# Improbable-AI/walk-these-ways

Measured on AMD Instinct MI355X. Metric: env-steps/sec (sim+PPO), higher is better.
Workload: dtype f32

## Files before the change

### include/go1ppo.h

```cpp
#ifndef GO1PPO_H
#define GO1PPO_H
#include <stdint.h>

#ifdef __cplusplus
extern "C" {
#endif

#define GO1PPO_ABI_VERSION 3
#define GO1PPO_MAX_ACTIONS 32

int go1ppo_elu_fwd(void* y, int64_t rows, int cols, int ld, const void* lat, int lat_ld, int npv, const void* wz,
                   int wz_ld, int lat_cols, void* stream);

int go1ppo_elu_bwd(const void* d, int ld_d, const void* h, int ld_h, int64_t rows, int cols, float* bias_grad, void* out,
                   int ld_out, void* stream);

typedef struct {
  const void* mean;
  const void* value;
  const float* std;
  int32_t head_ld, num_actions;
  int64_t rows;
  const int64_t* idx;
  const float* actions;
// ... 102 lines not shown
int go1ppo_opt_prestep_pieces(float* g, int64_t n, const Go1PpoGradPiece* device_pieces, int num_pieces, float gscale, float* partial,
                              float* step, float* lr, const float* kl, float kl_scale, float desired_kl, float lr_min, float lr_max,
                              void* stream);

#define GO1PPO_ADAM_MAX_TRANSPOSES 2
typedef struct {
  int32_t num_transposes, _pad;
  struct { int64_t start; int32_t rows, cols; void* dst; } transpose[GO1PPO_ADAM_MAX_TRANSPOSES];
} Go1PpoAdamExtras;
int go1ppo_opt_adam(float* p, float* g, float* m, float* v, int64_t start0, int64_t count0, int64_t start1,
                    int64_t count1, float gscale, const float* partial, float max_norm, const float* step, const float* lr,
                    float beta1, float beta2, float eps, void* body, int64_t n_body, float* tail, int64_t n_tail, int zero_grad,
                    float* zero_slot, const Go1PpoAdamExtras* extras, void* stream);

int go1ppo_sum_partials(const void* partials, int count, int64_t stride, int64_t rows, int cols, float* out, int zero_rows,
                        int zero_c0, int zero_c1, void* stream);


typedef struct Go1PpoGemmArgs {
  const void* A; const void* B; void* C; const float* bias; const void* H;
  int32_t M, N, K, lda, ldb, ldc, ldh, epilogue, elu_c0, elu_c1;
  int32_t elu_skip_c0, elu_skip_c1;
  int32_t bias_bf16, _pad;
} Go1PpoGemmArgs;
int go1ppo_gemm_nt(const Go1PpoGemmArgs* args, void* stream);
int go1ppo_gemm_nt_pair(const Go1PpoGemmArgs* a, const Go1PpoGemmArgs* b, void* stream);

int go1ppo_wgrad_tn_plan(Go1PpoWgradProblem* problems, int count);
int go1ppo_wgrad_tn_batched(const Go1PpoWgradProblem* device_problems, int count, int total_workgroups, void* stream);

#define GO1PPO_MLP2_MAX_NETS 3
typedef struct {
  void* x;
  const void* W2; const void* b2;
  const void* W3; const void* b3;
  void* z2;
  void* out;
  int64_t rows;
  int32_t ld_x, ld_z2, ld_out, elu_input;
} Go1PpoMlp2Fwd;
int go1ppo_mlp2_fwd(const Go1PpoMlp2Fwd* nets, int count, void* stream);

typedef struct {
  const void* d_out;
  const void* z2; const void* h;
  const void* W2; const void* W3;
  void* d_z2;
  void* d_x;
  int64_t rows;
  int32_t ld_dout, ld_z2, ld_h, ld_dz2, ld_dx, _pad;
} Go1PpoMlp2Bwd;
int go1ppo_mlp2_bwd(const Go1PpoMlp2Bwd* nets, int count, void* stream);

const char* go1ppo_version(void);

#ifdef __cplusplus
}
#endif
#endif
```

### walk-these-ways_amd/csrc/go1ppo.hip

```cpp
#include <hip/hip_runtime.h>
#include <stdint.h>
#include <string.h>
#include "../../include/go1ppo.h"

typedef uint16_t bf16_t;
static_assert(sizeof(Go1PpoAdamExtras) == 56 && sizeof(Go1PpoGemmArgs) == 96 && sizeof(Go1PpoWgradProblem) == 96 && sizeof(Go1PpoGradPiece) == 56, "ctypes mirrors (fused.py) assume these sizes");
typedef __attribute__((ext_vector_type(4))) float f32x4;

__device__ __forceinline__ float bf2f(bf16_t u) { return __uint_as_float(((uint32_t)u) << 16); }
__device__ __forceinline__ bf16_t f2bf(float f) {
  return __builtin_bit_cast(bf16_t, (__bf16)f);
}
struct alignas(16) Bf8 { bf16_t v[8]; };

__device__ __forceinline__ float elu1(float x) {
  float em = x > -1e-3f ? fmaf(0.5f * x, x, x) : __expf(x) - 1.f;
  return x > 0.f ? x : em;
}

typedef __attribute__((ext_vector_type(2))) float f32x2;
typedef __attribute__((ext_vector_type(2))) __bf16 bf16x2_t;
__device__ __forceinline__ Bf8 pack_bf8(const float (&x)[8]) {
  union { Bf8 b; uint32_t u[4]; } r;
#pragma unroll
  for (int e = 0; e < 4; e++) {
    f32x2 v = {x[2 * e], x[2 * e + 1]};
    r.u[e] = __builtin_bit_cast(uint32_t, __builtin_convertvector(v, bf16x2_t));
  }
  return r.b;
}

#ifndef ELU_ROWS
#define ELU_ROWS 4
#endif
template <bool LAT>
__global__ __launch_bounds__(256) void elu_fwd_kernel(bf16_t* y, int rows, int cols, int ld, const bf16_t* lat, int lat_ld,
                                                      int npv, const bf16_t* wz, int wz_ld, int lat_cols) {
  int c0 = (blockIdx.x * 16 + (threadIdx.x & 15)) << 3;
  int r0 = blockIdx.y * (16 * ELU_ROWS) + (threadIdx.x >> 4);
  if (c0 >= cols) return;
  Bf8 v[ELU_ROWS];
#pragma unroll
  for (int u = 0; u < ELU_ROWS; u++) {
    int r = r0 + u * 16;
    if (r < rows) v[u] = *reinterpret_cast<const Bf8*>(y + (int64_t)r * ld + c0);
  }
  float x[ELU_ROWS][8];
#pragma unroll
  for (int u = 0; u < ELU_ROWS; u++)
#pragma unroll
    for (int e = 0; e < 8; e++) x[u][e] = bf2f(v[u].v[e]);
  if (LAT && c0 < lat_cols) {
    if (npv == 2) {
      float w0[8], w1[8];
#pragma unroll
      for (int e = 0; e < 8; e++) {
        const uint32_t p = *reinterpret_cast<const uint32_t*>(wz + (int64_t)(c0 + e) * wz_ld);
        w0[e] = __uint_as_float(p << 16);
        w1[e] = __uint_as_float(p & 0xffff0000u);
// ... 1262 lines not shown
```

### walk-these-ways_amd/csrc/go1ppo_mlp.h

```cpp
#pragma once

#define MLP2_K1 256
#define MLP2_N2 128
#define MLP2_N3 64
#define MLP2_BM 64
#define MLP2_WAVES 16
#define MLP2_THREADS (64 * MLP2_WAVES)
#define MLP2_IMG (128 * 128)

struct Mlp2FwdArgs { Go1PpoMlp2Fwd net[GO1PPO_MLP2_MAX_NETS]; };
struct Mlp2BwdArgs { Go1PpoMlp2Bwd net[GO1PPO_MLP2_MAX_NETS]; };

__device__ __forceinline__ int swz_row(int row) { return row & 15; }
__device__ __forceinline__ int swz_red(int row) { return 2 * ((row & 3) | (((row >> 3) & 1) << 2)); }

template <bool RED>
__device__ __forceinline__ void dma_weights(const bf16_t* W, int rows, int cols, bf16_t* img, int wave, int lane) {
  const int windows = cols >> 7, count = (rows >> 2) * windows;
  for (int idx = wave; idx < count; idx += MLP2_WAVES) {
    const int win = idx % windows, blk = idx / windows;
    const int row = blk * 4 + (lane >> 4);
    const int chunk = (lane & 15) ^ (RED ? swz_red(row) : swz_row(row));
    glds16(W + (int64_t)row * cols + win * 128 + chunk * 8, img + win * MLP2_IMG + blk * 4 * 128);
  }
// ... 174 lines not shown
      f32x4 acc[2] = {f32x4{0.f, 0.f, 0.f, 0.f}, f32x4{0.f, 0.f, 0.f, 0.f}};
#pragma unroll
      for (int kk = 0; kk < MLP2_N3 / 32; kk++) {
        const bf16x8_t w = lds_tr_operand(W3t, kk * 32 * 256 + w3off);
#pragma unroll
        for (int m = 0; m < 2; m++) acc[m] = __builtin_amdgcn_mfma_f32_16x16x32_bf16(w, lds_b128(D3i + (mp + m) * 16 * 128, foff[kk]), acc[m], 0, 0, 0);
      }
      const int k0 = kf2 * 16 + 4 * g;
#pragma unroll
      for (int m = 0; m < 2; m++) {
        const int row = (mp + m) * 16 + r;
        uint2* slot = reinterpret_cast<uint2*>(reinterpret_cast<char*>(D2i) + row * 256 + (((k0 >> 3) ^ swz_row(row)) << 4) + ((k0 >> 2) & 1) * 8);
        float h[4], o4[4];
        unpack_bf4(*slot, h);
#pragma unroll
        for (int e = 0; e < 4; e++) o4[e] = acc[m][e] * (h[e] > 0.f ? 1.f : h[e] + 1.f);
        *slot = pack_bf4(o4);
      }
    }
    __syncthreads();
    {
      f32x4 acc[4];
#pragma unroll
      for (int m = 0; m < 4; m++) acc[m] = f32x4{0.f, 0.f, 0.f, 0.f};
#pragma unroll
      for (int kk = 0; kk < MLP2_N2 / 32; kk++) {
        const bf16x8_t w = lds_tr_operand(w2img, kk * 32 * 256 + w2off);
#pragma unroll
        for (int m = 0; m < 4; m++) acc[m] = __builtin_amdgcn_mfma_f32_16x16x32_bf16(w, lds_b128(D2i + m * 16 * 128, foff[kk]), acc[m], 0, 0, 0);
      }
      const int k0 = (wave & 7) * 16 + 4 * g;
#pragma unroll
      for (int m = 0; m < 4; m++) {
        const int row = m * 16 + r;
        uint2* slot = reinterpret_cast<uint2*>(reinterpret_cast<char*>(Hi + (wave >> 3) * 64 * 128) + row * 256 +
                                               (((k0 >> 3) ^ swz_row(row)) << 4) + ((k0 >> 2) & 1) * 8);
        float h[4], o4[4];
        unpack_bf4(*slot, h);
#pragma unroll
        for (int e = 0; e < 4; e++) o4[e] = acc[m][e] * (h[e] > 0.f ? 1.f : h[e] + 1.f);
        *slot = pack_bf4(o4);
      }
    }
    __syncthreads();
    if (row0 + zrow < N.rows) *reinterpret_cast<uint4*>(dz2 + (row0 + zrow) * N.ld_dz2 + zch * 8) = *reinterpret_cast<const uint4*>(reinterpret_cast<const char*>(D2i) + zslot);
#pragma unroll
    for (int j = 0; j < 2; j++)
      if (row0 + MLP2_HROW(j) < N.rows)
        *reinterpret_cast<uint4*>(dx + (row0 + MLP2_HROW(j)) * N.ld_dx + hch * 8) = *reinterpret_cast<const uint4*>(reinterpret_cast<const char*>(Hi) + MLP2_HSLOT(j));
    __syncthreads();
  }
}

static inline bool aligned8(const void* p) { return (reinterpret_cast<uintptr_t>(p) & 7) == 0; }

extern "C" int go1ppo_mlp2_fwd(const Go1PpoMlp2Fwd* nets, int count, void* stream) {
  if (!nets || count <= 0 || count > GO1PPO_MLP2_MAX_NETS) return -1;
  Mlp2FwdArgs A;
  int64_t max_rows = 0;
  for (int i = 0; i < count; i++) {
    const Go1PpoMlp2Fwd& N = nets[i];
    if (!N.x || !N.W2 || !N.b2 || !N.W3 || !N.b3 || !N.z2 || !N.out || N.rows <= 0) return -1;
    if ((N.ld_x & 7) || (N.ld_z2 & 3) || (N.ld_out & 3) || N.ld_x < MLP2_K1 || N.ld_z2 < MLP2_N2 || N.ld_out < MLP2_N3 || !aligned16(N.x) ||
        !aligned16(N.W2) || !aligned16(N.W3) || !aligned8(N.b2) || !aligned8(N.b3) || !aligned8(N.z2) || !aligned8(N.out))
      return -2;
    A.net[i] = N;
    if (N.rows > max_rows) max_rows = N.rows;
  }
  int64_t wgs = (max_rows + MLP2_BM - 1) / MLP2_BM;
  if (wgs > 256 / count) wgs = 256 / count;
  mlp2_fwd_kernel<<<dim3((unsigned)wgs, count), dim3(MLP2_THREADS), 0, (hipStream_t)stream>>>(A);
  return hipGetLastError() == hipSuccess ? 0 : -9;
}

extern "C" int go1ppo_mlp2_bwd(const Go1PpoMlp2Bwd* nets, int count, void* stream) {
  if (!nets || count <= 0 || count > GO1PPO_MLP2_MAX_NETS) return -1;
  Mlp2BwdArgs A;
  int64_t max_rows = 0;
  for (int i = 0; i < count; i++) {
    const Go1PpoMlp2Bwd& N = nets[i];
    if (!N.d_out || !N.z2 || !N.h || !N.W2 || !N.W3 || !N.d_z2 || !N.d_x || N.rows <= 0) return -1;
    if ((N.ld_dout & 7) || (N.ld_z2 & 7) || (N.ld_h & 7) || (N.ld_dz2 & 7) || (N.ld_dx & 7) || N.ld_dout < MLP2_N3 || N.ld_z2 < MLP2_N2 ||
        N.ld_h < MLP2_K1 || N.ld_dz2 < MLP2_N2 || N.ld_dx < MLP2_K1 || !aligned16(N.d_out) || !aligned16(N.W2) || !aligned16(N.W3) ||
        !aligned16(N.z2) || !aligned16(N.h) || !aligned16(N.d_z2) || !aligned16(N.d_x))
      return -2;
    A.net[i] = N;
    if (N.rows > max_rows) max_rows = N.rows;
  }
  int64_t wgs = (max_rows + MLP2_BM - 1) / MLP2_BM;
  if (wgs > 256 / count) wgs = 256 / count;
  mlp2_bwd_kernel<<<dim3((unsigned)wgs, count), dim3(MLP2_THREADS), 0, (hipStream_t)stream>>>(A);
  return hipGetLastError() == hipSuccess ? 0 : -9;
}
```

### walk-these-ways_amd/go1_gym_learn/ppo_cse/fused.py

```python
import ctypes
import os

import torch

HEAD = 64
_HERE = os.path.dirname(os.path.abspath(__file__))
_LIB_PATH = os.path.normpath(os.path.join(_HERE, "..", "..", "csrc", "libgo1ppo.so"))
_lib = None


class Go1PpoLibraryMissing(RuntimeError):
    pass


class LossArgs(ctypes.Structure):
    _fields_ = [("mean", ctypes.c_void_p), ("value", ctypes.c_void_p), ("std", ctypes.c_void_p),
                ("head_ld", ctypes.c_int32), ("num_actions", ctypes.c_int32), ("rows", ctypes.c_int64),
                ("idx", ctypes.c_void_p), ("actions", ctypes.c_void_p), ("old_mu", ctypes.c_void_p),
                ("old_sigma", ctypes.c_void_p), ("old_logp", ctypes.c_void_p), ("advantages", ctypes.c_void_p),
                ("returns", ctypes.c_void_p), ("old_values", ctypes.c_void_p),
                ("clip_param", ctypes.c_float), ("value_loss_coef", ctypes.c_float), ("entropy_coef", ctypes.c_float),
                ("use_clipped_value_loss", ctypes.c_int32),
                ("d_mean", ctypes.c_void_p), ("d_value", ctypes.c_void_p), ("d_std", ctypes.c_void_p),
                ("d_mean_bias", ctypes.c_void_p), ("d_value_bias", ctypes.c_void_p), ("kl", ctypes.c_void_p),
                ("value_loss", ctypes.c_void_p), ("surrogate_loss", ctypes.c_void_p)]


class WgradProblem(ctypes.Structure):
    _fields_ = [("dz", ctypes.c_void_p), ("h", ctypes.c_void_p), ("dW", ctypes.c_void_p), ("bias_grad", ctypes.c_void_p),
                ("rows", ctypes.c_int64), ("ld_dz", ctypes.c_int32), ("ld_h", ctypes.c_int32), ("n", ctypes.c_int32),
                ("k", ctypes.c_int32), ("ldw", ctypes.c_int32), ("chunk_rows", ctypes.c_int32), ("wg_offset", ctypes.c_int32),
                ("zero_n", ctypes.c_int32), ("zero_k0", ctypes.c_int32), ("zero_k1", ctypes.c_int32),
                ("partials", ctypes.c_void_p), ("partial_stride", ctypes.c_int64)]


class GradPiece(ctypes.Structure):
    _fields_ = [("begin", ctypes.c_int64), ("count", ctypes.c_int64), ("src", ctypes.c_void_p), ("stride", ctypes.c_int64),
                ("kind", ctypes.c_int32), ("slabs", ctypes.c_int32), ("cols", ctypes.c_int32), ("zero_rows", ctypes.c_int32),
                ("zero_c0", ctypes.c_int32), ("zero_c1", ctypes.c_int32)]


class TailLayer(ctypes.Structure):
    _fields_ = [("W", ctypes.c_void_p), ("bias", ctypes.c_void_p), ("out", ctypes.c_void_p), ("n_out", ctypes.c_int32),
                ("k_in", ctypes.c_int32), ("ld_out", ctypes.c_int32), ("elu", ctypes.c_int32)]


class TailNet(ctypes.Structure):
    _fields_ = [("in_", ctypes.c_void_p), ("rows", ctypes.c_int64), ("ld_in", ctypes.c_int32), ("num_layers", ctypes.c_int32),
                ("elu_in", ctypes.c_int32), ("npv", ctypes.c_int32), ("latent", ctypes.c_void_p), ("wz", ctypes.c_void_p),
                ("lat_ld", ctypes.c_int32), ("wz_ld", ctypes.c_int32),
                ("layer", TailLayer * 4)]


class TailArgs(ctypes.Structure):
    _fields_ = [("num_nets", ctypes.c_int32), ("_pad", ctypes.c_int32), ("net", TailNet * 3)]


class Mlp2Fwd(ctypes.Structure):
    _fields_ = [(n, ctypes.c_void_p) for n in ("x", "W2", "b2", "W3", "b3", "z2", "out")] + [("rows", ctypes.c_int64)] + \
               [(n, ctypes.c_int32) for n in ("ld_x", "ld_z2", "ld_out", "elu_input")]


class Mlp2Bwd(ctypes.Structure):
    _fields_ = [(n, ctypes.c_void_p) for n in ("d_out", "z2", "h", "W2", "W3", "d_z2", "d_x")] + [("rows", ctypes.c_int64)] + \
               [(n, ctypes.c_int32) for n in ("ld_dout", "ld_z2", "ld_h", "ld_dz2", "ld_dx", "_pad")]


MLP2_DIMS = (256, 128, 64)


class GemmArgs(ctypes.Structure):
    _fields_ = [("A", ctypes.c_void_p), ("B", ctypes.c_void_p), ("C", ctypes.c_void_p), ("bias", ctypes.c_void_p),
                ("H", ctypes.c_void_p)] + [(n, ctypes.c_int32) for n in
                                           ("M", "N", "K", "lda", "ldb", "ldc", "ldh", "epilogue", "elu_c0", "elu_c1", "elu_skip_c0", "elu_skip_c1", "bias_bf16", "_pad")]


class _AdamTranspose(ctypes.Structure):
    _fields_ = [("start", ctypes.c_int64), ("rows", ctypes.c_int32), ("cols", ctypes.c_int32), ("dst", ctypes.c_void_p)]


class AdamExtras(ctypes.Structure):
    _fields_ = [("num_transposes", ctypes.c_int32), ("_pad", ctypes.c_int32), ("transpose", _AdamTranspose * 2)]


EXPORTED_SYMBOLS = ["go1ppo_mlp2_fwd", "go1ppo_mlp2_bwd", "go1ppo_gemm_nt", "go1ppo_gemm_nt_pair", "go1ppo_sum_partials", "go1ppo_wgrad_tn_plan", "go1ppo_wgrad_tn_batched", "go1ppo_tail_fwd", "go1ppo_elu_fwd", "go1ppo_elu_bwd", "go1ppo_loss", "go1ppo_mse", "go1ppo_wgrad", "go1ppo_wgrad_plan",
                    "go1ppo_wgrad_batched", "go1ppo_act",
                    "go1ppo_store_step", "go1ppo_ring_snapshot", "go1ppo_ring_step", "go1ppo_ring_gather", "go1ppo_gae", "go1ppo_normalize", "go1ppo_opt_partials", "go1ppo_opt_prestep",
                    "go1ppo_opt_prestep_pieces", "go1ppo_grad_reduce", "go1ppo_opt_adam", "go1ppo_version"]


def load_library(path=None):
    global _lib
    if _lib is not None and path is None:
        return _lib
    p = path or _LIB_PATH
    if not os.path.exists(p):
        raise Go1PpoLibraryMissing(f"{p} not found: run `python -c 'import __graft_entry__ as g; g.build()'` "
                                   "(hipcc --offload-arch=gfx950); the fused PPO update has no CPU fallback")
    L = ctypes.CDLL(p)
    vp, i32, i64 = ctypes.c_void_p, ctypes.c_int, ctypes.c_int64
    L.go1ppo_elu_fwd.argtypes = [vp, i64, i32, i32, vp, i32, i32, vp, i32, i32, vp]
    L.go1ppo_elu_bwd.argtypes = [vp, i32, vp, i32, i64, i32, vp, vp, i32, vp]
    L.go1ppo_loss.argtypes = [ctypes.POINTER(LossArgs), vp]
    L.go1ppo_mse.argtypes = [vp, i32, vp, i32, vp, i64, i64, i32, vp, vp, vp, vp, vp]
    L.go1ppo_wgrad.argtypes = [vp, i32, vp, i32, i64, i32, i32, vp, i32, vp, vp]
    L.go1ppo_wgrad_plan.argtypes = [ctypes.POINTER(WgradProblem), i32]
    L.go1ppo_tail_fwd.argtypes = [ctypes.POINTER(TailArgs), vp]
    L.go1ppo_gemm_nt.argtypes = [ctypes.POINTER(GemmArgs), vp]
    L.go1ppo_gemm_nt_pair.argtypes = [ctypes.POINTER(GemmArgs), ctypes.POINTER(GemmArgs), vp]
    L.go1ppo_sum_partials.argtypes = [vp, i32, i64, i64, i32, vp, i32, i32, i32, vp]
    L.go1ppo_mlp2_fwd.argtypes = [ctypes.POINTER(Mlp2Fwd), i32, vp]
    L.go1ppo_mlp2_bwd.argtypes = [ctypes.POINTER(Mlp2Bwd), i32, vp]
    L.go1ppo_wgrad_batched.argtypes = [vp, i32, i32, vp]
    L.go1ppo_wgrad_tn_plan.argtypes = [ctypes.POINTER(WgradProblem), i32]
    L.go1ppo_wgrad_tn_batched.argtypes = [vp, i32, i32, vp]
    f32 = ctypes.c_float
    L.go1ppo_act.argtypes = [vp, vp, i32, vp, i32, i64, vp, vp, vp, vp, vp, vp, vp]
    L.go1ppo_store_step.argtypes = [vp, vp, vp, vp, vp, f32, i64, vp, vp, vp, vp]
    L.go1ppo_ring_snapshot.argtypes = [vp, i64, i64, i32, i32, vp, vp]
    L.go1ppo_ring_step.argtypes = [vp, vp, vp, vp, i64, i32, i32, i32, i32, vp, vp, vp, vp]
    L.go1ppo_ring_gather.argtypes = [vp, vp, vp, i64, i64, i32, i32, i32, i32, vp, vp]
    L.go1ppo_gae.argtypes = [vp, vp, vp, vp, i32, i64, f32, f32, vp, vp, vp, vp]
    L.go1ppo_normalize.argtypes = [vp, i64, vp, vp]
    L.go1ppo_opt_partials.argtypes = []
    L.go1ppo_opt_prestep.argtypes = [vp, i64, f32, vp, vp, vp, vp, f32, f32, f32, f32, vp]
    L.go1ppo_opt_prestep_pieces.argtypes = [vp, i64, vp, i32, f32, vp, vp, vp, vp, f32, f32, f32, f32, vp]
    L.go1ppo_grad_reduce.argtypes = [vp, vp, i32, vp]
    L.go1ppo_opt_adam.argtypes = [vp, vp, vp, vp, i64, i64, i64, i64, f32, vp, f32, vp, vp, f32, f32, f32, vp, i64, vp, i64, i32, vp,
                                  ctypes.POINTER(AdamExtras), vp]
    for name in EXPORTED_SYMBOLS[:-1]:
        getattr(L, name).restype = ctypes.c_int
    L.go1ppo_version.restype = ctypes.c_char_p
    if path is None:
        _lib = L
    return L


def _stream():
    return torch.cuda.current_stream().cuda_stream


def _chk(rc, what):
    if rc != 0:
        raise RuntimeError(f"{what} failed with code {rc}")


def _ptr(t):
    return None if t is None else t.data_ptr()


def _ld(t):
    assert t.dim() == 2 and t.stride(1) == 1
    return t.stride(0)


def gemm_args(a, b, c, bias=None, elu=None, elu_bwd_of=None, elu_skip=None):
    g = GemmArgs()
    g.A, g.B, g.C, g.bias, g.H = a.data_ptr(), b.data_ptr(), c.data_ptr(), _ptr(bias), _ptr(elu_bwd_of)
    g.M, g.N, g.K, g.lda, g.ldb, g.ldc = a.shape[0], b.shape[0], a.shape[1], _ld(a), _ld(b), _ld(c)
    assert b.shape[1] == g.K and tuple(c.shape) == (g.M, g.N) and (elu is None or elu_bwd_of is None)
    assert a.dtype == b.dtype == c.dtype == torch.bfloat16 and (bias is None or bias.dtype in (torch.float32, torch.bfloat16))
    g.bias_bf16 = int(bias is not None and bias.dtype == torch.bfloat16)
    if elu_bwd_of is not None:
        assert elu_bwd_of.shape == c.shape and elu_bwd_of.dtype == torch.bfloat16
        g.epilogue, g.ldh = 2, _ld(elu_bwd_of)
# ... 10 lines not shown
    _chk(lib.go1ppo_gemm_nt(ctypes.byref(g), _stream()), "go1ppo_gemm_nt")
    return c


def gemm_nt_pair(lib, first, second):
    ga, gb = gemm_args(**first), gemm_args(**second)
    _chk(lib.go1ppo_gemm_nt_pair(ctypes.byref(ga), ctypes.byref(gb), _stream()), "go1ppo_gemm_nt_pair")


class FusedNet:

    def __init__(self, policy, body, grad, M, lib, with_grad, two_streams=True, fused_tails=None):
        assert body.dtype == torch.bfloat16 and body.is_cuda
        self.pol, self.M, self.lib = policy, M, lib
        dev = body.device
        self.P = {name: policy._block(body, name) for name, _ in policy.blocks}
        self.G = {name: policy._block(grad, name) for name, _ in policy.blocks} if grad is not None else None
        self.nd, self.na, self.nc = policy.first
        self.n1 = self.nd + self.na + self.nc
        self.depth = {n: len(l) for n, l in policy.nets.items()}
        bf = dict(device=dev, dtype=torch.bfloat16)
        self.Y1 = torch.zeros(M, self.n1, **bf)
        self.Y1d = torch.zeros(M, self.nd, **bf)
        self.Z = {n: {li: torch.zeros(M, self.P[f"{n}.{li}.W"].shape[0], **bf) for li in range(1, d)}
                  for n, d in self.depth.items()}
        assert policy.npv <= HEAD and self.P["Wz"].shape == (self.na, HEAD)
        self._recording, self._batched, self._plans = None, False, {}
        self._grad = grad
        self.defer_grad_sum = False
        self._rec_pieces, self._slab_ws, self._last_pieces = None, {}, {}
        self._wgrad_tn = M % 64 == 0
        self._tails = self._tails_ad = None
        if fused_tails is None:
            fused_tails = M <= int(os.environ.get("GO1_FUSED_TAILS_MAX_ROWS", "2048"))
        self._elu_on_load = not with_grad
        if fused_tails and self._fused_tails_ok():
            nd, na = self.nd, self.na
            eol = self._elu_on_load
            self._tails = (self._tail_args([("adaptation", self.Y1[:, :nd])], with_grad, elu_in=eol),
                           self._tail_args([("actor", self.Y1[:, nd:nd + na]), ("critic", self.Y1[:, nd + na:])], with_grad, elu_in=eol,
                                           latent_for="actor" if eol else None))
            self._tails_ad = self._tail_args([("adaptation", self.Y1d)], with_grad)
        self._mlp2 = (self._tails is None and os.environ.get("GO1_MLP2", "1") == "1" and self.nd == MLP2_DIMS[0] and
                      all(self.depth[n] >= 3 and tuple(self.P[f"{n}.{self.depth[n] - 2}.W"].shape) == (MLP2_DIMS[1], MLP2_DIMS[0])
                          and tuple(self.P[f"{n}.{self.depth[n] - 1}.W"].shape) == (MLP2_DIMS[2], MLP2_DIMS[1]) for n in self.depth)
                      and self.depth["adaptation"] == 3 and self.depth["actor"] == 4 and self.depth["critic"] == 4)
        self._mlp2_cache = {}
        na1, nc1 = int(self.P["actor.1.W"].shape[0]), int(self.P["critic.1.W"].shape[0])
        nt_ok = all(v % 64 == 0 for v in (na1, nc1, self.na, self.n1 - self.nd - self.na)) and \
            all(self.P[k].data_ptr() % 16 == 0 for k in ("actor.1.b", "critic.1.b", "actor.1.W", "critic.1.W"))
        pair_ok = nt_ok and na1 == nc1 and self.na == self.n1 - self.nd - self.na
        self._l1_nt = nt_ok
        self._pair = pair_ok
        self._side = torch.cuda.Stream(device=dev) if two_streams else None
        if with_grad:
            self.X = torch.zeros(M, policy.Kp, **bf)
            self.dH1 = {"adaptation": torch.zeros(M, self.nd, **bf), "actor": torch.zeros(M, self.na, **bf),
                        "critic": torch.zeros(M, self.nc, **bf)}
            self.dY1 = torch.zeros(M, self.n1, **bf)
            self.dZ = {n: {li: torch.zeros_like(z) for li, z in zs.items()} for n, zs in self.Z.items()}
            w1_split = next((b for b in (M // 6144, 4, 2) if b >= 2 and M % b == 0 and (M // b) % 64 == 0), 1)
            self._w1_tmp = torch.zeros(w1_split, self.n1, policy.Kp, **bf)
            self._dgrad_nt = self._mlp2 and nt_ok
            self._WT = {n: torch.zeros(self.P[f"{n}.1.W"].shape[1], self.P[f"{n}.1.W"].shape[0], **bf) for n in ("actor", "critic")} \
                if self._dgrad_nt else None
            self._wt_by_optimizer = False
            self.priv_mask = (self.nd + self.na, policy.K + 1, policy.K + 1 + policy.npv)

    def _elu(self, y, lat=None, lat_cols=0):
        wz = self.P["Wz"] if lat is not None else None
        _chk(self.lib.go1ppo_elu_fwd(y.data_ptr(), y.shape[0], y.shape[1], _ld(y), _ptr(lat), _ld(lat) if lat is not None else 0,
                                     self.pol.npv if lat is not None else 0, _ptr(wz), HEAD, lat_cols, _stream()), "go1ppo_elu_fwd")

    def _elu_bwd(self, d, h, bias_grad, out=None):
        out = d if out is None else out
        _chk(self.lib.go1ppo_elu_bwd(d.data_ptr(), _ld(d), _ptr(h), _ld(h) if h is not None else 0, d.shape[0], d.shape[1],
                                     _ptr(bias_grad), out.data_ptr(), _ld(out), _stream()), "go1ppo_elu_bwd")

    def _wgrad(self, dz, h, gW, gb=None, zero=None):
        n, k = dz.shape[1], h.shape[1]
        assert gW.shape == (n, k) and gW.is_contiguous()
        if self._recording is not None:
            self._recording.append((dz, h, gW, gb, zero))
            return
        if self._batched:
            return
        assert zero is None or zero[0] == 0, "the structural zeros are applied by the batched launch"
        _chk(self.lib.go1ppo_wgrad(dz.data_ptr(), _ld(dz), h.data_ptr(), _ld(h), dz.shape[0], n, k, gW.data_ptr(), k, _ptr(gb),
                                   _stream()), "go1ppo_wgrad")

    def _tail_args(self, nets_and_inputs, keep_intermediates, elu_in=False, latent_for=None):
        a = TailArgs()
        a.num_nets = len(nets_and_inputs)
        for N, (net, h) in zip(a.net, nets_and_inputs):
            d = self.depth[net]
            N.in_, N.rows, N.ld_in, N.num_layers = h.data_ptr(), h.shape[0], _ld(h), d - 1
            N.elu_in = int(bool(elu_in))
            if elu_in and latent_for == net:
                lat, wz = self.Z["adaptation"][self.depth["adaptation"] - 1], self.P["Wz"]
                N.latent, N.wz, N.lat_ld, N.wz_ld, N.npv = lat.data_ptr(), wz.data_ptr(), _ld(lat), HEAD, self.pol.npv
            for li in range(1, d):
                L, W, z = N.layer[li - 1], self.P[f"{net}.{li}.W"], self.Z[net][li]
                last = li == d - 1
                L.W, L.bias = W.data_ptr(), self.P[f"{net}.{li}.b"].data_ptr()
                L.out = z.data_ptr() if (last or keep_intermediates) else None
                L.n_out, L.k_in, L.ld_out, L.elu = W.shape[0], W.shape[1], _ld(z), 0 if last else 1
# ... 23 lines not shown
            return self._forward_mlp2(x)
        torch.mm(x, self.P["W1"].t(), out=self.Y1)
        if self._tails is not None:
            ta, tac = self._tails
            if not self._elu_on_load:
                self._elu(self.Y1[:, :nd])
            _chk(self.lib.go1ppo_tail_fwd(ctypes.byref(ta), _stream()), "go1ppo_tail_fwd")
            latent = self.Z["adaptation"][self.depth["adaptation"] - 1]
            if not self._elu_on_load:
                self._elu(self.Y1[:, nd:], latent, na)
            _chk(self.lib.go1ppo_tail_fwd(ctypes.byref(tac), _stream()), "go1ppo_tail_fwd")
            return self.Z["actor"][self.depth["actor"] - 1], self.Z["critic"][self.depth["critic"] - 1], latent
        self._elu(self.Y1[:, :nd])
        latent = self._tail("adaptation", self.Y1[:, :nd])
        self._elu(self.Y1[:, nd:], latent, na)
        with self._branch():
            value = self._tail("critic", self.Y1[:, nd + na:])
        mean = self._tail("actor", self.Y1[:, nd:nd + na])
        self._join()
        return mean, value, latent

    def _mlp2_fwd(self, key, items, elu_input=1):
        key = ("fwd", key, elu_input)
        if key not in self._mlp2_cache:
            arr = (Mlp2Fwd * len(items))()
            for a, (net, x) in zip(arr, items):
                d = self.depth[net]
                W2, W3, z2, out = self.P[f"{net}.{d - 2}.W"], self.P[f"{net}.{d - 1}.W"], self.Z[net][d - 2], self.Z[net][d - 1]
                a.x, a.W2, a.b2, a.W3, a.b3 = x.data_ptr(), W2.data_ptr(), self.P[f"{net}.{d - 2}.b"].data_ptr(), W3.data_ptr(), self.P[f"{net}.{d - 1}.b"].data_ptr()
                a.z2, a.out, a.rows, a.ld_x, a.ld_z2, a.ld_out, a.elu_input = z2.data_ptr(), out.data_ptr(), x.shape[0], _ld(x), _ld(z2), _ld(out), int(elu_input)
            self._mlp2_cache[key] = (arr, len(items))
        arr, n = self._mlp2_cache[key]
        _chk(self.lib.go1ppo_mlp2_fwd(arr, n, _stream()), "go1ppo_mlp2_fwd")

    def _mlp2_bwd(self, key, items):
        key = ("bwd", key)
        if key not in self._mlp2_cache:
            arr = (Mlp2Bwd * len(items))()
            for a, (net, h, d_x) in zip(arr, items):
                d = self.depth[net]
                d_out, z2, d_z2 = self.dZ[net][d - 1], self.Z[net][d - 2], self.dZ[net][d - 2]
                a.d_out, a.z2, a.h, a.W2, a.W3 = d_out.data_ptr(), z2.data_ptr(), h.data_ptr(), self.P[f"{net}.{d - 2}.W"].data_ptr(), self.P[f"{net}.{d - 1}.W"].data_ptr()
                a.d_z2, a.d_x, a.rows = d_z2.data_ptr(), d_x.data_ptr(), h.shape[0]
                a.ld_dout, a.ld_z2, a.ld_h, a.ld_dz2, a.ld_dx = _ld(d_out), _ld(z2), _ld(h), _ld(d_z2), _ld(d_x)
            self._mlp2_cache[key] = (arr, len(items))
        arr, n = self._mlp2_cache[key]
        _chk(self.lib.go1ppo_mlp2_bwd(arr, n, _stream()), "go1ppo_mlp2_bwd")

    def _forward_mlp2(self, x):
        P, Z, nd, na = self.P, self.Z, self.nd, self.na
        torch.mm(x, P["W1"].t(), out=self.Y1)
        self._mlp2_fwd("adaptation", [("adaptation", self.Y1[:, :nd])])
        latent = Z["adaptation"][2]
        self._elu(self.Y1[:, nd:], latent, na)
        if self._l1_nt and self._pair:
            gemm_nt_pair(self.lib, dict(a=self.Y1[:, nd:nd + na], b=P["actor.1.W"], c=Z["actor"][1], bias=P["actor.1.b"]),
                         dict(a=self.Y1[:, nd + na:], b=P["critic.1.W"], c=Z["critic"][1], bias=P["critic.1.b"]))
        elif self._l1_nt:
            with self._branch():
                gemm_nt(self.lib, self.Y1[:, nd + na:], P["critic.1.W"], Z["critic"][1], P["critic.1.b"])
            gemm_nt(self.lib, self.Y1[:, nd:nd + na], P["actor.1.W"], Z["actor"][1], P["actor.1.b"])
        else:
            with self._branch():
                torch.addmm(P["critic.1.b"], self.Y1[:, nd + na:], P["critic.1.W"].t(), out=Z["critic"][1])
            torch.addmm(P["actor.1.b"], self.Y1[:, nd:nd + na], P["actor.1.W"].t(), out=Z["actor"][1])
        self._join()
        self._mlp2_fwd("ac", [("actor", Z["actor"][1]), ("critic", Z["critic"][1])])
        return Z["actor"][3], Z["critic"][3], latent

    def _backward_mlp2(self, x):
        nd, na = self.nd, self.na
        P, G, Z, dZ, Y1, dY1, dH1 = self.P, self.G, self.Z, self.dZ, self.Y1, self.dY1, self.dH1
        cols = {"adaptation": slice(0, nd), "actor": slice(nd, nd + na), "critic": slice(nd + na, self.n1)}
        self._mlp2_bwd("ac", [("actor", Z["actor"][1], dZ["actor"][1]), ("critic", Z["critic"][1], dZ["critic"][1])])
        for net in ("actor", "critic"):
            self._wgrad(dZ[net][3], Z[net][2], G[f"{net}.3.W"], None)
            self._wgrad(dZ[net][2], Z[net][1], G[f"{net}.2.W"], G[f"{net}.2.b"])
            self._wgrad(dZ[net][1], Y1[:, cols[net]], G[f"{net}.1.W"], G[f"{net}.1.b"])
        if self._dgrad_nt and self._pair and self._wt_by_optimizer:
            gemm_nt_pair(self.lib, dict(a=dZ["actor"][1], b=self._WT["actor"], c=dY1[:, cols["actor"]], elu_bwd_of=Y1[:, cols["actor"]]),
                         dict(a=dZ["critic"][1], b=self._WT["critic"], c=dY1[:, cols["critic"]], elu_bwd_of=Y1[:, cols["critic"]]))
        elif self._dgrad_nt:
            with self._branch():
                if not self._wt_by_optimizer:
                    self._WT["critic"].copy_(P["critic.1.W"].t())
                gemm_nt(self.lib, dZ["critic"][1], self._WT["critic"], dY1[:, cols["critic"]], elu_bwd_of=Y1[:, cols["critic"]])
            if not self._wt_by_optimizer:
                self._WT["actor"].copy_(P["actor.1.W"].t())
            gemm_nt(self.lib, dZ["actor"][1], self._WT["actor"], dY1[:, cols["actor"]], elu_bwd_of=Y1[:, cols["actor"]])
        else:
            with self._branch():
                torch.mm(dZ["critic"][1], P["critic.1.W"], out=dH1["critic"])
                self._elu_bwd(dH1["critic"], Y1[:, cols["critic"]], None, out=dY1[:, cols["critic"]])
            torch.mm(dZ["actor"][1], P["actor.1.W"], out=dH1["actor"])
            self._elu_bwd(dH1["actor"], Y1[:, cols["actor"]], None, out=dY1[:, cols["actor"]])
        latent, dlat = Z["adaptation"][2], dZ["adaptation"][2]
        dA1 = dY1[:, cols["actor"]]
        self._wgrad(dA1, latent, G["Wz"])
        torch.mm(dA1, P["Wz"], out=dlat)
        self._mlp2_bwd("adaptation", [("adaptation", Y1[:, :nd], dY1[:, :nd])])
        self._wgrad(dlat, Z["adaptation"][1], G["adaptation.2.W"], G["adaptation.2.b"])
        self._wgrad(dZ["adaptation"][1], Y1[:, :nd], G["adaptation.1.W"], G["adaptation.1.b"])
        self._join()
        self._big_wgrad(dY1, x, G["W1"], self._w1_tmp)

    def _forward_adaptation_mlp2(self, x):
        torch.mm(x, self.P["W1"][:self.nd].t(), out=self.Y1d)
        self._mlp2_fwd("adaptation_only", [("adaptation", self.Y1d)])
        return self.Z["adaptation"][2]

    def _backward_adaptation_mlp2(self, x):
        nd, d, G, Z, dZ = self.nd, self.dH1["adaptation"], self.G, self.Z, self.dZ
        self._mlp2_bwd("adaptation_only", [("adaptation", self.Y1d, d)])
        self._wgrad(dZ["adaptation"][2], Z["adaptation"][1], G["adaptation.2.W"], None)
        self._wgrad(dZ["adaptation"][1], self.Y1d, G["adaptation.1.W"], G["adaptation.1.b"])
        self._big_wgrad(d, x, G["W1"][:nd], self._w1_tmp[:, :nd], own_kernel=self._wgrad_tn)

    def adam_transposes(self):
        if not getattr(self, "_dgrad_nt", False):
            return []
        out = []
# ... 303 lines not shown
```

Baseline: 5.117 million.

## Fuse actor/critic ELU, layer-1 GEMM and MLP tail into one inference kernel

After: 5.156 million (median of 6 runs). No clear change (+0.8%).

```diff
diff --git a/include/go1ppo.h b/include/go1ppo.h
--- a/include/go1ppo.h
+++ b/include/go1ppo.h
@@ -178,6 +178,23 @@
 } Go1PpoMlp2Bwd;
 int go1ppo_mlp2_bwd(const Go1PpoMlp2Bwd* nets, int count, void* stream);
 
+#define GO1PPO_AC_MAX_NETS 2
+typedef struct {
+  void* y1;
+  const void* W1; const void* b1;
+  const void* W2; const void* b2;
+  const void* W3; const void* b3;
+  void* z1;
+  void* z2;
+  void* out;
+  const void* latent;
+  const void* wz;
+  int64_t rows;
+  int32_t ld_y1, ld_z1, ld_z2, ld_out, lat_ld, wz_ld, npv;
+  int32_t store_act;
+} Go1PpoAcFwd;
+int go1ppo_ac_fwd(const Go1PpoAcFwd* nets, int count, void* stream);
+
 const char* go1ppo_version(void);
 
 #ifdef __cplusplus
diff --git a/walk-these-ways_amd/csrc/go1ppo.hip b/walk-these-ways_amd/csrc/go1ppo.hip
--- a/walk-these-ways_amd/csrc/go1ppo.hip
+++ b/walk-these-ways_amd/csrc/go1ppo.hip
@@ -4,7 +4,7 @@
 #include "../../include/go1ppo.h"
 
 typedef uint16_t bf16_t;
-static_assert(sizeof(Go1PpoAdamExtras) == 56 && sizeof(Go1PpoGemmArgs) == 96 && sizeof(Go1PpoWgradProblem) == 96 && sizeof(Go1PpoGradPiece) == 56, "ctypes mirrors (fused.py) assume these sizes");
+static_assert(sizeof(Go1PpoAdamExtras) == 56 && sizeof(Go1PpoAcFwd) == 136 && sizeof(Go1PpoGemmArgs) == 96 && sizeof(Go1PpoWgradProblem) == 96 && sizeof(Go1PpoGradPiece) == 56, "ctypes mirrors (fused.py) assume these sizes");
 typedef __attribute__((ext_vector_type(4))) float f32x4;
 
 __device__ __forceinline__ float bf2f(bf16_t u) { return __uint_as_float(((uint32_t)u) << 16); }
diff --git a/walk-these-ways_amd/csrc/go1ppo_mlp.h b/walk-these-ways_amd/csrc/go1ppo_mlp.h
--- a/walk-these-ways_amd/csrc/go1ppo_mlp.h
+++ b/walk-these-ways_amd/csrc/go1ppo_mlp.h
@@ -250,6 +250,223 @@
   }
 }
 
+#define ACF_BM 64
+#define ACF_K1 512
+#define ACF_N1 256
+#define ACF_KC 64
+#define ACF_CHUNKS (ACF_K1 / ACF_KC)
+__device__ __forceinline__ int opaque_lane(int x) {
+  asm volatile("" : "+v"(x));
+  return x;
+}
+struct AcFwdArgs { Go1PpoAcFwd net[GO1PPO_AC_MAX_NETS]; };
+
+__global__ __launch_bounds__(MLP2_THREADS, 1) void ac_fwd_kernel(AcFwdArgs A) {
+  __shared__ __attribute__((aligned(1024))) bf16_t W2i[2 * MLP2_IMG];
+  __shared__ __attribute__((aligned(1024))) bf16_t W3i[64 * 128];
+  __shared__ __attribute__((aligned(1024))) bf16_t S[2 * ACF_N1 * ACF_KC + 2 * ACF_BM * ACF_KC];
+  bf16_t* const Wc0 = S;
+  bf16_t* const Ac0 = S + 2 * ACF_N1 * ACF_KC;
+  bf16_t* const Z1i = S + ACF_N1 * ACF_KC;
+  bf16_t* const Z2i = Ac0;
+  const Go1PpoAcFwd& N = A.net[blockIdx.y];
+  const int tiles = (int)((N.rows + ACF_BM - 1) / ACF_BM);
+  if ((int)blockIdx.x >= tiles) return;
+  const int t = threadIdx.x, wave = t >> 6, lane = t & 63, r = lane & 15, g = lane >> 4;
+  dma_weights<false>((const bf16_t*)N.W2, MLP2_N2, MLP2_K1, W2i, wave, lane);
+  dma_weights<false>((const bf16_t*)N.W3, MLP2_N3, MLP2_N2, W3i, wave, lane);
+  bf16_t* y1 = (bf16_t*)N.y1;
+  const bf16_t* W1 = (const bf16_t*)N.W1;
+  const bf16_t* lat = (const bf16_t*)N.latent;
+  const bf16_t* wz = (const bf16_t*)N.wz;
+  const bool store = N.store_act != 0;
+
+  const bf16_t* gw[2];
+#pragma unroll
+  for (int p = 0; p < 2; p++) {
+    const int R = (wave * 2 + p) * 8 + (lane >> 3);
+    gw[p] = W1 + (int64_t)R * ACF_K1 + (((lane & 7) ^ ((R >> 1) & 7)) << 3);
+  }
+  auto stage_w1 = [&](int buf, int kc) {
+#pragma unroll
+    for (int p = 0; p < 2; p++) glds16(gw[p] + kc * ACF_KC, Wc0 + buf * ACF_N1 * ACF_KC + (wave * 2 + p) * 8 * ACF_KC);
+  };
+  const int ar = (t >> 3) & 63, ach = t & 7;
+  const bool apiece = t < 512;
+  Bf8 va;
+  uint32_t latp = 0, wzp[8];
+  auto fetch_a = [&](int tile, int kc) {
+    if (!apiece) return;
+    int64_t grow = (int64_t)tile * ACF_BM + ar;
+    grow = grow < N.rows ? grow : N.rows - 1;
+    va = *reinterpret_cast<const Bf8*>(y1 + grow * N.ld_y1 + kc * ACF_KC + opaque_lane(ach) * 8);
+    if (lat && N.npv == 2) {
+      if (kc == 0) latp = *reinterpret_cast<const uint32_t*>(lat + grow * N.lat_ld);
+#pragma unroll
+      for (int e = 0; e < 8; e++) wzp[e] = *reinterpret_cast<const uint32_t*>(wz + (int64_t)(kc * ACF_KC + ach * 8 + e) * N.wz_ld);
+    }
+  };
+  int foff1[2];
+#pragma unroll
+  for (int kk = 0; kk < 2; kk++) foff1[kk] = r * ACF_KC + (((kk * 4 + g) ^ (r >> 1)) << 3);
+  const int nfb = (wave >> 1) * 2, mfb = (wave & 1) * 2;
+  uint2 b1raw[2];
+#pragma unroll
+  for (int j = 0; j < 2; j++) b1raw[j] = *reinterpret_cast<const uint2*>((const bf16_t*)N.b1 + (nfb + j) * 16 + 4 * g);
+
+  const int tx = g ^ r;
+  int foff[4];
+#pragma unroll
+  for (int a = 0; a < 4; a++) foff[a] = r * 256 + (((4 * a) ^ tx) << 4);
+  const int nf2 = wave >> 1, mp = (wave & 1) * 2, nf3 = wave & 3, m3 = wave >> 2;
+  const uint2 b2raw = *reinterpret_cast<const uint2*>((const bf16_t*)N.b2 + nf2 * 16 + 4 * g);
+  const uint2 b3raw = *reinterpret_cast<const uint2*>((const bf16_t*)N.b3 + nf3 * 16 + 4 * g);
+  bf16_t* z1 = (bf16_t*)N.z1;
+  bf16_t* z2 = (bf16_t*)N.z2;
+  bf16_t* out = (bf16_t*)N.out;
+
+  stage_w1(0, 0);
+  fetch_a(blockIdx.x, 0);
+  for (int tile = blockIdx.x; tile < tiles; tile += gridDim.x) {
+    const int64_t row0 = (int64_t)tile * ACF_BM;
+    f32x4 acc1[2][2];
+#pragma unroll
+    for (int j = 0; j < 2; j++)
+#pragma unroll
+      for (int i = 0; i < 2; i++) acc1[j][i] = f32x4{0.f, 0.f, 0.f, 0.f};
+#pragma unroll 1
+    for (int kc = 0; kc < ACF_CHUNKS; kc++) {
+      const int buf = kc & 1;
+      __builtin_amdgcn_s_waitcnt(0x0f70);
+      if (apiece) {
+        float f[8];
+#pragma unroll
+        for (int e = 0; e < 8; e++) f[e] = bf2f(va.v[e]);
+        if (lat) {
+          if (N.npv == 2) {
+            const float l0 = __uint_as_float(latp << 16), l1 = __uint_as_float(latp & 0xffff0000u);
+#pragma unroll
+            for (int e = 0; e < 8; e++) f[e] = fmaf(l1, __uint_as_float(wzp[e] & 0xffff0000u), fmaf(l0, __uint_as_float(wzp[e] << 16), f[e]));
+          } else {
+            int64_t grow = row0 + ar;
+            grow = grow < N.rows ? grow : N.rows - 1;
+            for (int q = 0; q < N.npv; q++) {
+              const float l = bf2f(lat[grow * N.lat_ld + q]);
+#pragma unroll
+              for (int e = 0; e < 8; e++) f[e] = fmaf(l, bf2f(wz[(int64_t)(kc * ACF_KC + ach * 8 + e) * N.wz_ld + q]), f[e]);
+            }
+          }
+        }
+#pragma unroll
+        for (int e = 0; e < 8; e++) f[e] = elu1(f[e]);
+        const Bf8 h = pack_bf8(f);
+        if (store && row0 + ar < N.rows) *reinterpret_cast<Bf8*>(y1 + (row0 + ar) * N.ld_y1 + kc * ACF_KC + ach * 8) = h;
+        *reinterpret_cast<Bf8*>(Ac0 + buf * ACF_BM * ACF_KC + ar * ACF_KC + ((ach ^ ((ar >> 1) & 7)) << 3)) = h;
+      }
+      __syncthreads();
+      if (kc + 1 < ACF_CHUNKS) {
+        stage_w1(buf ^ 1, kc + 1);
+        fetch_a(tile, kc + 1);
+      }
+      const bf16_t* wb = Wc0 + buf * ACF_N1 * ACF_KC + nfb * 16 * ACF_KC;
+      const bf16_t* ab = Ac0 + buf * ACF_BM * ACF_KC + mfb * 16 * ACF_KC;
+#pragma unroll
+      for (int kk = 0; kk < 2; kk++) {
+        bf16x8_t w[2], x[2];
+#pragma unroll
+        for (int j = 0; j < 2; j++) w[j] = *reinterpret_cast<const bf16x8_t*>(wb + j * 16 * ACF_KC + foff1[kk]);
+#pragma unroll
+        for (int i = 0; i < 2; i++) x[i] = *reinterpret_cast<const bf16x8_t*>(ab + i * 16 * ACF_KC + foff1[kk]);
+#pragma unroll
+        for (int j = 0; j < 2; j++)
+#pragma unroll
+          for (int i = 0; i < 2; i++) acc1[j][i] = __builtin_amdgcn_mfma_f32_16x16x32_bf16(w[j], x[i], acc1[j][i], 0, 0, 0);
+      }
+    }
+    __syncthreads();
+#pragma unroll
+    for (int j = 0; j < 2; j++) {
+      const int n = (nfb + j) * 16 + 4 * g, nw = n & 127;
+#pragma unroll
+      for (int i = 0; i < 2; i++) {
+        const int row = (mfb + i) * 16 + r;
+        float v[4], bias1[4];
+        uint2 braw = b1raw[j];
+        asm volatile("" : "+v"(braw.x), "+v"(braw.y));
+        unpack_bf4(braw, bias1);
+#pragma unroll
+        for (int e = 0; e < 4; e++) v[e] = acc1[j][i][e] + bias1[e];
+        unpack_bf4(pack_bf4(v), v);
+#pragma unroll
+        for (int e = 0; e < 4; e++) v[e] = elu1(v[e]);
+        *reinterpret_cast<uint2*>(reinterpret_cast<char*>(Z1i + (n >> 7) * 64 * 128) + row * 256 + (((nw >> 3) ^ swz_row(row)) << 4) +
+                                  ((nw >> 2) & 1) * 8) = pack_bf4(v);
+      }
+    }
+    __syncthreads();
+    if (tile + (int)gridDim.x < tiles) {
+      stage_w1(0, 0);
+      fetch_a(tile + gridDim.x, 0);
+    }
+    if (store) {
+#pragma unroll
+      for (int j = 0; j < 2; j++) {
+        const int p = t + MLP2_THREADS * j, row = p >> 5, ch = p & 31;
+        const int gch = opaque_lane(ch);
+        if (row0 + row < N.rows)
+          *reinterpret_cast<uint4*>(z1 + (row0 + row) * N.ld_z1 + gch * 8) =
+              *reinterpret_cast<const uint4*>(reinterpret_cast<const char*>(Z1i) + (ch >> 4) * (64 * 128 * 2) + row * 256 + (((ch & 15) ^ swz_row(row)) << 4));
+      }
+    }
+    {
+      f32x4 acc[2] = {f32x4{0.f, 0.f, 0.f, 0.f}, f32x4{0.f, 0.f, 0.f, 0.f}};
+#pragma unroll 2
+      for (int ks = 0; ks < MLP2_K1 / 32; ks++) {
+        const int win = ks >> 2, off = foff[ks & 3];
+        const bf16x8_t w = lds_b128(W2i + win * MLP2_IMG + nf2 * 16 * 128, off);
+#pragma unroll
+        for (int m = 0; m < 2; m++)
+          acc[m] = __builtin_amdgcn_mfma_f32_16x16x32_bf16(w, lds_b128(Z1i + win * 64 * 128 + (mp + m) * 16 * 128, off), acc[m], 0, 0, 0);
+      }
+      const int n0 = nf2 * 16 + 4 * g;
+      float bias2[4];
+      uint2 braw = b2raw;
+      asm volatile("" : "+v"(braw.x), "+v"(braw.y));
+      unpack_bf4(braw, bias2);
+#pragma unroll
+      for (int m = 0; m < 2; m++) {
+        const int row = (mp + m) * 16 + r;
+        float o4[4];
+#pragma unroll
+        for (int e = 0; e < 4; e++) o4[e] = elu1(acc[m][e] + bias2[e]);
+        *reinterpret_cast<uint2*>(reinterpret_cast<char*>(Z2i) + row * 256 + (((n0 >> 3) ^ swz_row(row)) << 4) + ((n0 >> 2) & 1) * 8) = pack_bf4(o4);
+      }
+    }
+    __syncthreads();
+    if (store) {
+      const int row = t >> 4, ch = t & 15, gch = opaque_lane(ch);
+      if (row0 + row < N.rows)
+        *reinterpret_cast<uint4*>(z2 + (row0 + row) * N.ld_z2 + gch * 8) =
+            *reinterpret_cast<const uint4*>(reinterpret_cast<const char*>(Z2i) + row * 256 + ((ch ^ swz_row(row)) << 4));
+    }
+    {
+      f32x4 acc = f32x4{0.f, 0.f, 0.f, 0.f};
+#pragma unroll
+      for (int ks = 0; ks < MLP2_N2 / 32; ks++)
+        acc = __builtin_amdgcn_mfma_f32_16x16x32_bf16(lds_b128(W3i + nf3 * 16 * 128, foff[ks]), lds_b128(Z2i + m3 * 16 * 128, foff[ks]), acc, 0, 0, 0);
+      const int n0 = nf3 * 16 + 4 * g, row = m3 * 16 + r;
+      float o4[4], bias3[4];
+      uint2 braw = b3raw;
+      asm volatile("" : "+v"(braw.x), "+v"(braw.y));
+      unpack_bf4(braw, bias3);
+#pragma unroll
+      for (int e = 0; e < 4; e++) o4[e] = acc[e] + bias3[e];
+      if (row0 + row < N.rows) *reinterpret_cast<uint2*>(out + (row0 + row) * N.ld_out + opaque_lane(n0)) = pack_bf4(o4);
+    }
+    __syncthreads();
+  }
+}
+
 static inline bool aligned8(const void* p) { return (reinterpret_cast<uintptr_t>(p) & 7) == 0; }
 
 extern "C" int go1ppo_mlp2_fwd(const Go1PpoMlp2Fwd* nets, int count, void* stream) {
@@ -290,3 +507,30 @@
   mlp2_bwd_kernel<<<dim3((unsigned)wgs, count), dim3(MLP2_THREADS), 0, (hipStream_t)stream>>>(A);
   return hipGetLastError() == hipSuccess ? 0 : -9;
 }
+
+extern "C" int go1ppo_ac_fwd(const Go1PpoAcFwd* nets, int count, void* stream) {
+  if (!nets || count <= 0 || count > GO1PPO_AC_MAX_NETS) return -1;
+  AcFwdArgs A;
+  int64_t max_rows = 0;
+  for (int i = 0; i < count; i++) {
+    const Go1PpoAcFwd& N = nets[i];
+    if (!N.y1 || !N.W1 || !N.b1 || !N.W2 || !N.b2 || !N.W3 || !N.b3 || !N.out || N.rows <= 0 || N.rows > INT32_MAX ||
+        (N.store_act && (!N.z1 || !N.z2)) || (N.latent && (!N.wz || N.npv <= 0)))
+      return -1;
+    if ((N.ld_y1 & 7) || N.ld_y1 < ACF_K1 || (N.ld_out & 3) || N.ld_out < MLP2_N3 || !aligned16(N.y1) || !aligned16(N.W1) || !aligned16(N.W2) ||
+        !aligned16(N.W3) || !aligned8(N.b1) || !aligned8(N.b2) || !aligned8(N.b3) || !aligned8(N.out))
+      return -2;
+    if (N.store_act && ((N.ld_z1 & 7) || (N.ld_z2 & 7) || N.ld_z1 < ACF_N1 || N.ld_z2 < MLP2_N2 || !aligned16(N.z1) || !aligned16(N.z2)))
+      return -2;
+    if (N.latent && (N.lat_ld < N.npv || N.wz_ld < N.npv ||
+                     (N.npv == 2 && ((N.lat_ld & 1) || (N.wz_ld & 1) || ((uintptr_t)N.latent & 3) || ((uintptr_t)N.wz & 3)))))
+      return -2;
+    A.net[i] = N;
+    if (!N.latent) A.net[i].npv = 0;
+    if (N.rows > max_rows) max_rows = N.rows;
+  }
+  int64_t wgs = (max_rows + ACF_BM - 1) / ACF_BM;
+  if (wgs > 256 / count) wgs = 256 / count;
+  ac_fwd_kernel<<<dim3((unsigned)wgs, count), dim3(MLP2_THREADS), 0, (hipStream_t)stream>>>(A);
+  return hipGetLastError() == hipSuccess ? 0 : -9;
+}
diff --git a/walk-these-ways_amd/go1_gym_learn/ppo_cse/fused.py b/walk-these-ways_amd/go1_gym_learn/ppo_cse/fused.py
--- a/walk-these-ways_amd/go1_gym_learn/ppo_cse/fused.py
+++ b/walk-these-ways_amd/go1_gym_learn/ppo_cse/fused.py
@@ -69,6 +69,15 @@
 MLP2_DIMS = (256, 128, 64)
 
 
+class AcFwd(ctypes.Structure):
+    _fields_ = [(n, ctypes.c_void_p) for n in ("y1", "W1", "b1", "W2", "b2", "W3", "b3", "z1", "z2", "out", "latent", "wz")] + \
+               [("rows", ctypes.c_int64)] + \
+               [(n, ctypes.c_int32) for n in ("ld_y1", "ld_z1", "ld_z2", "ld_out", "lat_ld", "wz_ld", "npv", "store_act")]
+
+
+AC_FWD_DIMS = (512, 256)
+
+
 class GemmArgs(ctypes.Structure):
     _fields_ = [("A", ctypes.c_void_p), ("B", ctypes.c_void_p), ("C", ctypes.c_void_p), ("bias", ctypes.c_void_p),
                 ("H", ctypes.c_void_p)] + [(n, ctypes.c_int32) for n in
@@ -83,7 +92,7 @@
     _fields_ = [("num_transposes", ctypes.c_int32), ("_pad", ctypes.c_int32), ("transpose", _AdamTranspose * 2)]
 
 
-EXPORTED_SYMBOLS = ["go1ppo_mlp2_fwd", "go1ppo_mlp2_bwd", "go1ppo_gemm_nt", "go1ppo_gemm_nt_pair", "go1ppo_sum_partials", "go1ppo_wgrad_tn_plan", "go1ppo_wgrad_tn_batched", "go1ppo_tail_fwd", "go1ppo_elu_fwd", "go1ppo_elu_bwd", "go1ppo_loss", "go1ppo_mse", "go1ppo_wgrad", "go1ppo_wgrad_plan",
+EXPORTED_SYMBOLS = ["go1ppo_ac_fwd", "go1ppo_mlp2_fwd", "go1ppo_mlp2_bwd", "go1ppo_gemm_nt", "go1ppo_gemm_nt_pair", "go1ppo_sum_partials", "go1ppo_wgrad_tn_plan", "go1ppo_wgrad_tn_batched", "go1ppo_tail_fwd", "go1ppo_elu_fwd", "go1ppo_elu_bwd", "go1ppo_loss", "go1ppo_mse", "go1ppo_wgrad", "go1ppo_wgrad_plan",
                     "go1ppo_wgrad_batched", "go1ppo_act",
                     "go1ppo_store_step", "go1ppo_ring_snapshot", "go1ppo_ring_step", "go1ppo_ring_gather", "go1ppo_gae", "go1ppo_normalize", "go1ppo_opt_partials", "go1ppo_opt_prestep",
                     "go1ppo_opt_prestep_pieces", "go1ppo_grad_reduce", "go1ppo_opt_adam", "go1ppo_version"]
@@ -111,6 +120,7 @@
     L.go1ppo_sum_partials.argtypes = [vp, i32, i64, i64, i32, vp, i32, i32, i32, vp]
     L.go1ppo_mlp2_fwd.argtypes = [ctypes.POINTER(Mlp2Fwd), i32, vp]
     L.go1ppo_mlp2_bwd.argtypes = [ctypes.POINTER(Mlp2Bwd), i32, vp]
+    L.go1ppo_ac_fwd.argtypes = [ctypes.POINTER(AcFwd), i32, vp]
     L.go1ppo_wgrad_batched.argtypes = [vp, i32, i32, vp]
     L.go1ppo_wgrad_tn_plan.argtypes = [ctypes.POINTER(WgradProblem), i32]
     L.go1ppo_wgrad_tn_batched.argtypes = [vp, i32, i32, vp]
@@ -227,6 +237,12 @@
         pair_ok = nt_ok and na1 == nc1 and self.na == self.n1 - self.nd - self.na
         self._l1_nt = nt_ok
         self._pair = pair_ok
+        y1ac = self.Y1[:, self.nd:]
+        self._ac_fwd = (not with_grad and self._mlp2 and pair_ok and (self.na, na1) == AC_FWD_DIMS and
+                        tuple(self.P["actor.1.W"].shape) == tuple(self.P["critic.1.W"].shape) == (AC_FWD_DIMS[1], AC_FWD_DIMS[0]) and
+                        y1ac.data_ptr() % 16 == 0 and _ld(y1ac) % 8 == 0 and
+                        all(self.P[f"{n}.{li}.W"].data_ptr() % 16 == 0 and self.P[f"{n}.{li}.b"].data_ptr() % 8 == 0
+                            for n in ("actor", "critic") for li in (1, 2, 3)))
         self._side = torch.cuda.Stream(device=dev) if two_streams else None
         if with_grad:
             self.X = torch.zeros(M, policy.Kp, **bf)
@@ -356,6 +372,9 @@
         torch.mm(x, P["W1"].t(), out=self.Y1)
         self._mlp2_fwd("adaptation", [("adaptation", self.Y1[:, :nd])])
         latent = Z["adaptation"][2]
+        if self._ac_fwd:
+            self._ac_fwd_launch()
+            return Z["actor"][3], Z["critic"][3], latent
         self._elu(self.Y1[:, nd:], latent, na)
         if self._l1_nt and self._pair:
             gemm_nt_pair(self.lib, dict(a=self.Y1[:, nd:nd + na], b=P["actor.1.W"], c=Z["actor"][1], bias=P["actor.1.b"]),
@@ -371,6 +390,24 @@
         self._join()
         self._mlp2_fwd("ac", [("actor", Z["actor"][1]), ("critic", Z["critic"][1])])
         return Z["actor"][3], Z["critic"][3], latent
+
+    def _ac_fwd_launch(self):
+        if "ac_fwd" not in self._mlp2_cache:
+            nd, na, P, Z = self.nd, self.na, self.P, self.Z
+            latent, wz = Z["adaptation"][2], P["Wz"]
+            arr = (AcFwd * 2)()
+            for a, net, y in zip(arr, ("actor", "critic"), (self.Y1[:, nd:nd + na], self.Y1[:, nd + na:])):
+                a.y1, a.rows, a.ld_y1 = y.data_ptr(), y.shape[0], _ld(y)
+                a.W1, a.b1 = P[f"{net}.1.W"].data_ptr(), P[f"{net}.1.b"].data_ptr()
+                a.W2, a.b2 = P[f"{net}.2.W"].data_ptr(), P[f"{net}.2.b"].data_ptr()
+                a.W3, a.b3 = P[f"{net}.3.W"].data_ptr(), P[f"{net}.3.b"].data_ptr()
+                a.z1, a.z2, a.out = Z[net][1].data_ptr(), Z[net][2].data_ptr(), Z[net][3].data_ptr()
+                a.ld_z1, a.ld_z2, a.ld_out = _ld(Z[net][1]), _ld(Z[net][2]), _ld(Z[net][3])
+                a.store_act = 0
+                if net == "actor" and self.pol.npv > 0:
+                    a.latent, a.wz, a.lat_ld, a.wz_ld, a.npv = latent.data_ptr(), wz.data_ptr(), _ld(latent), HEAD, self.pol.npv
+            self._mlp2_cache["ac_fwd"] = arr
+        _chk(self.lib.go1ppo_ac_fwd(self._mlp2_cache["ac_fwd"], 2, _stream()), "go1ppo_ac_fwd")
 
     def _backward_mlp2(self, x):
         nd, na = self.nd, self.na
```
